# yeyupiaoling/MASR

Measured on AMD Instinct MI355X. Metric: audio-seconds/sec (RTF^-1), conformer_streaming_fbank b32x10s, PCM->fbank->encoder->ctc_greedy->text, higher is better.
Workload: dtype f32; 1 GPU; configs[1]: conformer.yml streaming fbank, batch=32 synthetic 16 kHz 10 s utterances per GPU, ctc_greedy, random-init weights V=4233; global_batch=32, parallelism=dp1, world_size_observed=1, backend=none

## Files before the change

### masr_amd/csrc/common.h

```cpp
#pragma once
#include <hip/hip_runtime.h>
#include <stdint.h>

#include "lm_scorer.h"

#ifndef MASR_EXPERIMENTS
#define MASR_EXPERIMENTS 0
#endif

typedef float f32x4 __attribute__((ext_vector_type(4)));
typedef float f32x16 __attribute__((ext_vector_type(16)));

namespace masr {

struct LdsAttr {
    size_t granted[32] = {};
};
void ensure_dynamic_lds(const void* fn, size_t bytes, LdsAttr& st);
void note_launch_error(const char* what, hipError_t e);

#ifdef __HIPCC__
struct SeqRow {
    int b, t;
};
// ... 173 lines not shown
    float eps;
};
struct FfnTail {
    const float* lnw;
    const float* lnb;
    const float* W;
    const float* bias;
    float* out;
    int N, ldo;
    const float* pre_lnw;
    const float* pre_lnb;
    long plane_stride;
    int seq_t, pad_t;
};
struct FfnHead {
    const float* glu;
    const float* dw_w;
    const float* dw_b;
    const float* lnw;
    const float* lnb;
    const float* gconst;
    const float* W;
    const float* bias;
    const int* lens;
    int seq_t, ktaps, mstride;
    float* xout;
};
int launch_ffn_fused(float* x, const float* lnw, const float* lnb, const float* w1, const float* b1, const float* w2,
                     const float* b2, int M, int dff, float eps, float scale, int affine_prologue, float* partial,
                     int nsplit, hipStream_t s, const FfnPostLn* post = nullptr, const FfnTail* tail = nullptr,
                     const FfnHead* head = nullptr, bool packed = false);
void launch_pack_ffn_pc(const float* w1, const float* w2, float* p1, float* p2, int dff, hipStream_t s);
void launch_pack_rows_pc(const float* w, float* p, int N, hipStream_t s, int n_src = -1);
int launch_ffn16(float* x, const float* lnw, const float* lnb, const float* w1, const float* b1, const float* w2, const float* b2, int M,
                 int dff, float eps, float scale, hipStream_t s, const FfnTail* tail, const FfnHead* head);
void launch_pack_ffn16(const float* w1, const float* w2, float* p1, float* p2, int dff, hipStream_t s);
void launch_pack_rows16(const float* w, float* p, int N, hipStream_t s, int n_src = -1);
struct SqzStageArgs {
    float* x;
    float* out;
    const float* att;
    const float* head_w;
    const float* head_b;
    const float *ln_a_w, *ln_a_b, *ln_b_w, *ln_b_b;
    const float *ffn_s, *ffn_b, *w1, *b1, *w2, *b2;
    const float *tail_w, *tail_b, *tail_s, *tail_sb;
    float* tail_out;
    float* glu_out;
    const float* glu;
    const float *dw_w, *dw_b, *bn_scale, *bn_shift, *gconst;
    const float* gpad;
    const int* lens;
    int M, dff, seq_t, mstride, ktaps, tail_n, glu_pad_l, glu_pad_tot;
    float eps;
    int skip_pad;
};
bool launch_sqz_stage(const SqzStageArgs& a, int stage, hipStream_t s);
#if MASR_EXPERIMENTS
int launch_ffn_dual(float* x, const float* lnw, const float* lnb, const float* p1, const float* b1, const float* p2,
                    const float* b2, int M, int dff, float eps, float scale, int affine_prologue, hipStream_t s,
                    const FfnTail* tail, const FfnHead* head);
void launch_pack_ffn_dual(const float* w1, const float* w2, float* p1, float* p2, int dff, hipStream_t s);
void launch_pack_rows_dual(const float* w, float* p, hipStream_t s);
#else
inline int launch_ffn_dual(float*, const float*, const float*, const float*, const float*, const float*, const float*, int, int, float,
                           float, int, hipStream_t, const FfnTail*, const FfnHead*) { return -1; }
inline void launch_pack_ffn_dual(const float*, const float*, float*, float*, int, hipStream_t) {}
inline void launch_pack_rows_dual(const float*, float*, hipStream_t) {}
// ... 131 lines not shown
```

### masr_amd/csrc/engine.hip

```cpp
#include <math.h>
#include <stdio.h>
#include <stdlib.h>
#include <string.h>

#include <map>
#include <mutex>
#include <string>
#include <vector>

#include "../../include/masr_hip.h"
#include "common.h"

using namespace masr;
namespace masr {
int lm_device_view(masr_lm* lm, LmView* out);
bool lm_word_based(const masr_lm* lm);
}
extern "C" const char* masr_lm_last_error(void);

static thread_local std::string g_err;
static int fail(const std::string& m) {
    g_err = m;
    return 1;
}
// ... 1030 lines not shown
        if (want_head) {
            phead = *head;
            CHK(p16(head->W, d, &phead.W));
        }
        const int done = launch_ffn16(e->x.as<float>(), lnw, lnb, it->second.first.as<float>(), b1, it->second.second.as<float>(), b2, M,
                                      dff, 1e-5f, scale, s, want_tail ? &ptail : nullptr, want_head ? &phead : nullptr);
        if (done < 0) return fail("ffn(): the 16-row FFN kernel rejected the launch");
        if (want_head && done != 4) return fail("ffn(): head stage was not launched");
        if (tail_done) *tail_done = done == 2;
        if (post_y) launch_layernorm(e->x.as<float>(), post_w, post_b, post_y, M, 1e-5f, 0, 0, nullptr, s);
        return 0;
    }
    if (packed && want_tail && tail->N % 256 == 0) {
        ptail = *tail;
        CHK(packed_rows(tail->W, tail->N, &ptail.W));
        tail = &ptail;
    }
    if (packed && want_head) {
        phead = *head;
        CHK(packed_rows(head->W, d, &phead.W));
        if (split_head) {
            CHK(e->xh.ensure((size_t)M * d * sizeof(float)));
            phead.xout = e->xh.as<float>();
        }
        head = &phead;
    }
    const int done = launch_ffn_fused(e->x.as<float>(), lnw, lnb, kw1, b1, kw2, b2, M, dff, 1e-5f, scale, affine,
                                      nsplit > 1 ? e->ffpart.as<float>() : nullptr, nsplit, s, post_y ? &post : nullptr,
                                      want_tail ? tail : nullptr, want_head ? head : nullptr, packed);
    if (done < 0) return fail("ffn(): launch rejected");
    if (want_head && !(done & 4)) return fail("ffn(): head stage was not launched");
    if (tail_done) *tail_done = done == 2;
    if (post_y && !(done & 1)) launch_layernorm(e->x.as<float>(), post_w, post_b, post_y, M, 1e-5f, 0, 0, nullptr, s);
    return 0;
}

static int g_hot_weights = 0;
static int g_embed_split = 1;
static int subsampling_conv(masr_engine* e, hipStream_t s, GemmArgs a, int amode, int nseq, const float* feats, const float* x_in) {
    const int d = e->cfg.d_model;
    const int tiles = ((a.M + 63) / 64) * ((a.N + 63) / 64);
    if (tiles >= 640 && g_conv2_rows && a.N == 256) {
        auto it = e->conv2_packed.find(a.W);
        if (it == e->conv2_packed.end()) {
            std::pair<DevBuf, DevBuf> pk;
            CHK(pk.first.ensure((size_t)a.N * a.K * sizeof(float)));
            launch_pack_conv2_rows(a.W, pk.first.as<float>(), a.K, s);
            it = e->conv2_packed.emplace(a.W, pk).first;
        }
        a.Wp = it->second.first.as<float>();
        if (feats && amode == A_CONV2 && g_conv1_fused && !g_bf16x3 && gemm_conv2_rows(a)) {
            a.feats = feats; a.mean = e->cmvn_mean; a.istd = e->cmvn_istd; a.c1w = e->conv1_w; a.c1b = e->conv1_b;
            a.Fin = e->cfg.n_mels;
        }
    }
    if (!a.feats) {
        if (feats) {
            CHK(e->x1.ensure((size_t)nseq * a.T1 * a.F1 * d * sizeof(float)));
            launch_conv1(feats, e->cmvn_mean, e->cmvn_istd, e->conv1_w, e->conv1_b, e->x1.as<float>(), nseq, a.Tin, e->cfg.n_mels,
                         d, s);
            a.A = e->x1.as<float>();
        } else {
            a.A = x_in;
        }
    }
    ProfScope ps(e, s, PROF_CONV2, 2.0 * a.M * (double)a.N * a.K);
// ... 713 lines not shown
    if (Tq_out) *Tq_out = Tq;
    return 0;
}

extern "C" {

int masr_encode_full(masr_engine* e, const float* feats_dev, const int32_t* feat_lens_dev, int32_t B, int32_t T,
                     int32_t decoding_chunk_size, float* enc_out_dev, void* stream) {
    if (!e || !e->finalized) return fail("engine not finalized");
    ENTER(e);
    CallGuard call_guard(e, (hipStream_t)stream);
    if (B <= 0) return fail("empty batch");
    hipStream_t s = (hipStream_t)stream;
    if (e->cfg.model_kind == 3) return ds2_forward(e, s, feats_dev, feat_lens_dev, B, T, enc_out_dev, nullptr, nullptr);
    const int chunk = (decoding_chunk_size > 0 && e->cfg.causal) ? decoding_chunk_size : 0;
    if (feat_lens_dev && e->input_layer != IL_CONV2D && !(feat_lens_dev = sub_lens(e, s, feat_lens_dev, B)))
        return fail("out of device memory (subsampled lengths)");
    if (e->cfg.model_kind == 1) return encode_full_squeezeformer(e, s, feats_dev, feat_lens_dev, B, T, enc_out_dev, chunk);
    if (e->cfg.model_kind == 2) return encode_full_efficient(e, s, feats_dev, feat_lens_dev, B, T, enc_out_dev, chunk);
    const int d = e->cfg.d_model, H = e->cfg.heads, pad = e->cfg.cnn_kernel - 1;
    int Tq = 0;
    CHK(embed(e, s, feats_dev, B, T, &Tq));
    if (Tq >= e->cfg.max_pos) return fail("sequence longer than max_pos");
    const int M = B * Tq;
    CHK(ensure_layer_ws(e, B, Tq));
    CHK(e->attseq.ensure(sizeof(AttSeq) * B));
    float* x = e->x.as<float>();
    EncodeCtx ctx{B, Tq, feat_lens_dev};
    launch_attseq_full(e->attseq.as<AttSeq>(), e->qkv.as<float>(), e->att.as<float>(), feat_lens_dev, B, Tq, 4, s);
    if (!e->cfg.causal)
        HIPCHK(hipMemsetAsync(e->glu.p, 0, (size_t)B * (Tq + pad) * d * sizeof(float), s));
    const LayerW* prev = nullptr;
    const bool few_rows = g_few_rows_path && (M + 31) / 32 < std::min(rowgemm_small_blocks(), g_ffn_split_blocks);
    for (const LayerW& w : e->layers) {
        const FfnTail tail{w.ln_mha_w, w.ln_mha_b, w.wqkv, w.bqkv, e->qkv.as<float>(), 3 * d, 3 * d,
                           prev ? prev->ln_fin_w : nullptr, prev ? prev->ln_fin_b : nullptr};
        bool qkv_done = false;
        CHK(ffn(e, s, M, w.ln_ffm_w, w.ln_ffm_b, w.ffm_w1, w.ffm_b1, w.ffm_w2, w.ffm_b2, 0.5f, 0, nullptr, nullptr, nullptr, &tail,
                &qkv_done));
        if (!qkv_done) mhsa(e, s, w, M);
        const bool fuse_ac = g_attn_chain && !few_rows && !g_no_chain && !e->conv_bn && H == 4 && d == 256 && g_rowgemm_packed;
        if (fuse_ac) {
            AttnChainArgs a{};
            a.seqs = e->attseq.as<AttSeq>(); a.nseq = B; a.q_stride = 3 * d; a.kv_stride = 3 * d;
            a.chunk_size = (decoding_chunk_size > 0 && e->cfg.causal) ? decoding_chunk_size : 0; a.pos_stride = 1;
            a.ptab = w.ptab; a.bias_u = w.pos_u; a.bias_v = w.pos_v;
            a.Wp = packed_rows_of(e, w.chain_w, 3 * d, s); a.bias = w.chain_b; a.lnw = w.ln_conv_w; a.lnb = w.ln_conv_b;
            a.R = x; a.R2 = x; a.C = e->glu.as<float>(); a.lens = feat_lens_dev; a.seq_t = Tq; a.mstride = 4;
            a.out_pad_l = e->cfg.causal ? pad : pad / 2; a.out_pad_tot = pad; a.eps = 1e-5f;
            if (!a.Wp) return fail("packed chain weights: allocation failed");
            ProfScope ps(e, s, PROF_ATT, 6.0 * d * (double)Tq * Tq * B + 2.0 * M * (double)(3 * d) * d);
            launch_attn_chain(a, Tq, s);
        } else {
            ProfScope ps(e, s, PROF_ATT, 6.0 * d * (double)Tq * Tq * B);
            launch_attention(e->attseq.as<AttSeq>(), B, Tq, H, 3 * d, 3 * d, w.ptab, w.pos_u, w.pos_v,
                             (decoding_chunk_size > 0 && e->cfg.causal) ? decoding_chunk_size : 0, 1, s);
        }
        if (few_rows) {
            mhsa_out(e, s, w, M);
            const bool fuse = g_split_head && e->cfg.cnn_kernel == 15 && g_ffn_packed >= 2 && !g_no_ffn_head && !e->conv_bn;
            CHK(conv_module(e, s, w, ctx, false, 0, 4, false, fuse));
            const FfnHead head{e->glu.as<float>(), w.dw_w, w.dw_b, w.cln_w, w.cln_b, e->cfg.causal ? w.gconst : nullptr,
                               w.pw2_w, w.pw2_b, feat_lens_dev, Tq, e->cfg.cnn_kernel, 4, nullptr};
            CHK(ffn(e, s, M, w.ln_ff_w, w.ln_ff_b, w.ff_w1, w.ff_b1, w.ff_w2, w.ff_b2, 0.5f, 0, w.ln_fin_w, w.ln_fin_b, x, nullptr,
                    nullptr, fuse ? &head : nullptr));
            continue;
        } else if (g_no_chain || e->conv_bn) {
            mhsa_out(e, s, w, M);
            CHK(conv_module(e, s, w, ctx, false));
            CHK(ffn(e, s, M, w.ln_ff_w, w.ln_ff_b, w.ff_w1, w.ff_b1, w.ff_w2, w.ff_b2));
        } else {
            if (!fuse_ac) mhsa_out_pw1(e, s, w, ctx);
            const FfnHead head{e->glu.as<float>(), w.dw_w, w.dw_b, w.cln_w, w.cln_b, e->cfg.causal ? w.gconst : nullptr,
                               w.pw2_w, w.pw2_b, feat_lens_dev, Tq, e->cfg.cnn_kernel, 4, nullptr};
            CHK(ffn(e, s, M, w.ln_ff_w, w.ln_ff_b, w.ff_w1, w.ff_b1, w.ff_w2, w.ff_b2, 0.5f, 0, nullptr, nullptr, nullptr, nullptr,
                    nullptr, &head));
        }
        prev = &w;
    }
    if (prev) launch_layernorm(x, prev->ln_fin_w, prev->ln_fin_b, x, M, 1e-5f, 0, 0, nullptr, s);
    launch_layernorm(x, e->after_w, e->after_b, enc_out_dev, M, 1e-5f, 0, 0, nullptr, s);
    LAUNCHCHK();
    return 0;
}

static int g_ctc_fused_blocks = 160;
static int ctc_head(masr_engine* e, const float* enc_dev, int M, float* probs_dev, int write_probs, int32_t* argmax_dev,
                    float* maxprob_dev, hipStream_t s) {
    const int d = enc_dim(e), V = e->cfg.vocab_size;
    float* logits = probs_dev;
    if (!logits) {
        CHK(e->logits.ensure((size_t)M * V * sizeof(float)));
        logits = e->logits.as<float>();
    }
    gemm(e, s, enc_dev, d, e->ctc_w, e->ctc_b, logits, V, M, V, d, ACT_NONE, 1.f, nullptr, 0);
    launch_softmax_argmax(logits, M, V, V, write_probs, argmax_dev, maxprob_dev, s);
    LAUNCHCHK();
    return 0;
}

int masr_ctc_probs(masr_engine* e, const float* enc_dev, int32_t M, float* probs_dev, int32_t* argmax_dev,
                   float* maxprob_dev, void* stream) {
    if (!e || !e->finalized) return fail("engine not finalized");
    ENTER(e);
    CallGuard call_guard(e, (hipStream_t)stream);
    if (!probs_dev) return fail("probs_dev is null");
    if (e->cfg.vocab_size > 16384) return fail("vocab_size > 16384 is not supported by the softmax / pruning kernels (one 256-thread workgroup holds a row in registers)");
    return ctc_head(e, enc_dev, M, probs_dev, 1, argmax_dev, maxprob_dev, (hipStream_t)stream);
}

int masr_ctc_greedy_frames(masr_engine* e, const float* enc_dev, int32_t M, int32_t* argmax_dev, float* maxprob_dev,
                           void* stream) {
    if (!e || !e->finalized) return fail("engine not finalized");
    ENTER(e);
// ... 1009 lines not shown
        return fail("masr_debug_set: this key selects an experimental kernel that is not in this build (MASR_BUILD_EXPERIMENTS=1)");
#endif
    if (key == 1) set_ffn_variant(value);
    else if (key == 5) g_no_chain = value;
    else if (key == 6) set_rowgemm_small(value);
    else if (key == 7) set_attention_fewq(value);
    else if (key == 14) set_attention_fold(value);
    else if (key == 15) g_embed_split = value;
    else if (key == 19) g_hot_weights = value;
    else if (key == 20) g_bf16x3 = value;
    else if (key == 21) set_gemm_bf16x3_waves(value);
    else if (key == 22) set_ffn_x3_rotation(value);
    else if (key == 23) g_ffn_packed = value;
    else if (key == 24) g_ffn_dual = value;
    else if (key == 25) g_rowgemm_packed = value;
    else if (key == 26) set_attention_grouped_fold(value);
    else if (key == 27) g_ctc_fused_blocks = value;
    else if (key == 28) set_attention_fewq_wgs(value);
    else if (key == 29) g_few_rows_path = value;
    else if (key == 30) g_split_head = value;
    else if (key == 31) g_efficient_fused = value;
    else if (key == 32) g_beam_lm_cache = value;
    else if (key == 33) set_conv2_mid_fill(value);
    else if (key == 34) g_attn_chain = value;
    else if (key == 35) g_ffn_coop = value;
    else if (key == 36) g_sqz_fused_blocks = value;
    else if (key == 37) g_beam_narrow = value;
    else if (key == 38) e->skip_padding = value;
    else if (key == 39) g_ffn16 = value;
    else if (key == 40) g_conv2_rows = value;
    else if (key == 41) g_conv1_fused = value;
    else if (key == 42) g_embed_rows = value;
    else if (key == 43) set_gru_mfma_units(value);
    else if (key == 17) set_gemm_waves(value);
    else if (key == 18) set_conv1_nt(value);
    else if (key == 16) { e->prof_stride = value > 1 ? value : 1; e->prof_seen = 0; }
    else if (key == 8) g_no_ffn_tail = value;
    else if (key == 9) g_no_ffn_head = value;
    else if (key == 12) set_rowgemm_small_blocks(value);
    else if (key == 13) g_ffn_split_blocks = value;
    else if (key == 2) {
        if (value) {
            if (!e->beam_prof) {
                void* p = nullptr;
                HIPCHK(hipMalloc(&p, 16 * sizeof(long long)));
                e->owned.push_back(p);
                e->beam_prof = (long long*)p;
            }
        } else if (e->beam_prof) {
            long long h[16];
            HIPCHK(hipMemcpy(h, e->beam_prof, sizeof(h), hipMemcpyDeviceToHost));
            fprintf(stderr, "beam phases (cycles, last workgroup): setup+hash %lld  extensions %lld  prefixes+count %lld  select %lld  compact %lld\n",
                    h[0], h[1], h[2], h[3], h[4]);
            fprintf(stderr, "  narrow step (%lld frames): tables+candidates %lld  hash+contexts %lld  children+scorer table %lld  extensions %lld  "
                    "prefixes+select %lld  scan %lld  survivors %lld  new prefixes %lld\n", h[5], h[6], h[7], h[8], h[9], h[10], h[11], h[12], h[13]);
            if (h[15] > 0) fprintf(stderr, "  wide step (%lld frames): %.1f distinct scorer contexts per frame\n", h[15], (double)h[14] / (double)h[15]);
            e->beam_prof = nullptr;
        }
    }
    else return fail("unknown debug key");
    return 0;
}

int masr_profile_select(masr_engine* e, int32_t kind) {
    if (!e) return fail("null engine");
    e->prof_kind = kind;
// ... 25 lines not shown
```

### masr_amd/csrc/ffn_pc.hip

```cpp
#include "common.h"

namespace masr {

static constexpr int PC_BM = 32;
static constexpr int PC_D = 256;
static constexpr int PC_CH = 128;
static constexpr int PC_XLD = PC_D + 4;
static constexpr int PC_HLD = PC_CH + 4;
static constexpr int PC_WLD = 32 + 4;
static constexpr int PC_WSLAB = 32 * PC_WLD;
static constexpr int PC_NSET = 4;
#ifdef PC_NOFENCE_PACKED
#define PC_FENCE(var) do { if ((var) != 2) __builtin_amdgcn_sched_barrier(0); } while (0)
#else
#define PC_FENCE(var) __builtin_amdgcn_sched_barrier(0)
#endif

#ifndef PC_BUFLOAD
#define PC_BUFLOAD 1
#endif
__device__ __forceinline__ f32x4 pc_bufld(__amdgpu_buffer_rsrc_t rs, unsigned lane16, unsigned float_index) {
    return __builtin_bit_cast(f32x4, __builtin_amdgcn_raw_buffer_load_b128(rs, lane16, float_index * 4u, 0));
}

// ... 489 lines not shown
                        } else if ((slot & 1) == 0) {
                            pre[pset][(slot - 8) >> 1] = *reinterpret_cast<const f32x4*>(
                                tsrc(t + (j + 1 + PC_NSET) / 8, (j + 1 + PC_NSET) & 7, (slot - 8) >> 1));
                        }
                        __builtin_amdgcn_sched_barrier(0);
                    }
                }
            }
            if (col < tail.N && tail.plane_stride > 0) {
                float* plane = tail.out + (size_t)t * tail.plane_stride + wave * 32 + frow;
                const int pb0 = row0 / tail.seq_t, pt0 = row0 - pb0 * tail.seq_t;
#pragma unroll
                for (int r = 0; r < 16; ++r) {
                    const int lr = (r & 3) + 8 * (r >> 2) + 4 * fh;
                    const SeqRow q = seq_row(pb0, pt0, tail.seq_t, lr);
                    if (row0 + lr < M) plane[((size_t)q.b * (tail.seq_t + tail.pad_t) + q.t) * 256] = acc[r] + bv;
                }
            } else if (col < tail.N) {
#pragma unroll
                for (int r = 0; r < 16; ++r) {
                    const int row = row0 + (r & 3) + 8 * (r >> 2) + 4 * fh;
                    if (row < M) tail.out[(size_t)row * tail.ldo + col] = acc[r] + bv;
                }
            }
        }
    }
}


static constexpr int P16_BM = 16;
static constexpr int P16_RING = 8;
__host__ __device__ constexpr int p16_k0(int kk) { return (kk & 1) * 4 + (kk >> 1); }

template <int TAIL, int HEADK>
__global__ __launch_bounds__(512) __attribute__((amdgpu_waves_per_eu(4))) void ffn16_kernel(
    float* x, const float* __restrict__ lnw, const float* __restrict__ lnb, const float* __restrict__ w1, const float* __restrict__ b1,
    const float* __restrict__ w2, const float* __restrict__ b2, int M, int dff, float eps, float scale, FfnTail tail, FfnHead head) {
    extern __shared__ __align__(16) float sm[];
    float* xn = sm;
    float* hs = xn + P16_BM * PC_XLD;

    const int tid = threadIdx.x, lane = tid & 63;
    const int wave = __builtin_amdgcn_readfirstlane(tid >> 6);
    const int role = wave >> 2, idx = wave & 3;
    const int row0 = blockIdx.x * P16_BM;
    const int fr = lane & 15, kk = lane >> 4, ko = p16_k0(kk);
    const unsigned lane16 = lane * 16;
    f32x4 pre[P16_RING];
    const float* xa = xn + fr * PC_XLD + ko;

    f32x4 gw_head = {0.f, 0.f, 0.f, 0.f}, gb_head = gw_head;
    if (HEADK > 0) {
        {
            constexpr int KT = HEADK > 0 ? HEADK : 1, pad = KT - 1;
            const int c = tid & 255, half = tid >> 8;
            float w[KT], win[KT], nw[8];
#pragma unroll
            for (int j = 0; j < KT; ++j) w[j] = head.dw_w[j * 256 + c];
            const float bv = head.dw_b[c];
            const float gc = head.gconst ? head.gconst[c] : 0.f;
            const bool has_gc = head.gconst != nullptr;
            const int hb0 = row0 / head.seq_t, ht0 = row0 - hb0 * head.seq_t, lr_last = M - 1 - row0;
#pragma unroll
            for (int rr = 0; rr < 8; ++rr) {
                const SeqRow q = seq_row(hb0, ht0, head.seq_t, min(half * 8 + rr, lr_last));
                nw[rr] = head.glu[((size_t)q.b * (pad + head.seq_t) + q.t + pad) * 256 + c];
            }
#pragma unroll
            for (int j = 0; j < KT; ++j) win[j] = 0.f;
#pragma unroll
// ... 30 lines not shown
                f32x4 o;
                o[0] = d0 * rstd * ww[0] + bb[0];
                o[1] = d1 * rstd * ww[1] + bb[1];
                o[2] = d2 * rstd * ww[2] + bb[2];
                o[3] = d3 * rstd * ww[3] + bb[3];
#pragma unroll
                for (int i = 0; i < 4; ++i) o[i] = o[i] / (1.0f + expf(-o[i]));
                *reinterpret_cast<f32x4*>(&xn[lr * PC_XLD + lane * 4]) = o;
            }
        }
        const __amdgpu_buffer_rsrc_t hrs = __builtin_amdgcn_make_buffer_rsrc(const_cast<float*>(head.W), 0, PC_D * PC_D * 4, 0x00020000);
        auto hld = [&](int f) -> f32x4 { return pc_bufld(hrs, lane16, (unsigned)(wave * 32 + f) * 256u); };
#pragma unroll
        for (int k = 0; k < P16_RING; ++k) pre[k] = hld(k);
        __syncthreads();
        {
            float bv[2], res[8];
            unsigned padded = 0;
            const int mb0 = row0 / head.seq_t, mt0 = row0 - mb0 * head.seq_t;
#pragma unroll
            for (int nt = 0; nt < 2; ++nt) {
                const int col = wave * 32 + 16 * nt + fr;
                bv[nt] = head.bias[col];
#pragma unroll
                for (int r = 0; r < 4; ++r) {
                    const int lrc = min(4 * kk + r, M - 1 - row0);
                    res[4 * nt + r] = x[(size_t)(row0 + lrc) * PC_D + col];
                    if (head.lens) {
                        const SeqRow q = seq_row(mb0, mt0, head.seq_t, lrc);
                        if (head.mstride * q.t >= head.lens[q.b]) padded |= 1u << (4 * nt + r);
                    }
                }
            }
            gw_head = *reinterpret_cast<const f32x4*>(lnw + lane * 4);
            gb_head = *reinterpret_cast<const f32x4*>(lnb + lane * 4);
            f32x4 acc[2] = {{0.f, 0.f, 0.f, 0.f}, {0.f, 0.f, 0.f, 0.f}};
            float a0 = xa[0], a1 = xa[2];
#pragma unroll
            for (int g = 0; g < 32; ++g) {
                float n0 = 0.f, n1 = 0.f;
                if (g + 1 < 32) { n0 = xa[8 * (g + 1)]; n1 = xa[8 * (g + 1) + 2]; }
#pragma unroll
                for (int q = 0; q < 4; ++q) {
                    acc[q & 1] = __builtin_amdgcn_mfma_f32_16x16x4f32(q < 2 ? a0 : a1, pre[g % P16_RING][q], acc[q & 1], 0, 0, 0);
                    if (q == 3 && g + P16_RING < 32) pre[g % P16_RING] = hld(g + P16_RING);
                    __builtin_amdgcn_sched_barrier(0);
                }
                a0 = n0;
                a1 = n1;
            }
            __syncthreads();
#pragma unroll
            for (int nt = 0; nt < 2; ++nt) {
                const int col = wave * 32 + 16 * nt + fr;
#pragma unroll
                for (int r = 0; r < 4; ++r) {
                    const int lr = 4 * kk + r;
                    float v = acc[nt][r] + bv[nt];
                    if (padded & (1u << (4 * nt + r))) v = 0.f;
                    v = res[4 * nt + r] + v;
                    if (row0 + lr < M) x[(size_t)(row0 + lr) * PC_D + col] = v;
                    xn[lr * PC_XLD + col] = v;
                }
            }
        }
        __syncthreads();
    }

    {
        const f32x4 gw = HEADK > 0 ? gw_head : *reinterpret_cast<const f32x4*>(lnw + lane * 4);
        const f32x4 gb = HEADK > 0 ? gb_head : *reinterpret_cast<const f32x4*>(lnb + lane * 4);
        f32x4 v4[2];
#pragma unroll
        for (int rr = 0; rr < 2; ++rr) {
            const int row = min(row0 + wave * 2 + rr, M - 1);
            v4[rr] = HEADK > 0 ? *reinterpret_cast<const f32x4*>(&xn[(wave * 2 + rr) * PC_XLD + lane * 4])
                               : *reinterpret_cast<const f32x4*>(x + (size_t)row * PC_D + lane * 4);
        }
        if (TAIL && tail.pre_lnw) {
            const f32x4 pw = *reinterpret_cast<const f32x4*>(tail.pre_lnw + lane * 4);
            const f32x4 pb = *reinterpret_cast<const f32x4*>(tail.pre_lnb + lane * 4);
#pragma unroll
            for (int rr = 0; rr < 2; ++rr) {
                const f32x4 v = v4[rr];
                const float mean = pc_wsum(v[0] + v[1] + v[2] + v[3]) * (1.0f / 256.0f);
                const float d0 = v[0] - mean, d1 = v[1] - mean, d2 = v[2] - mean, d3 = v[3] - mean;
                const float var = pc_wsum(d0 * d0 + d1 * d1 + d2 * d2 + d3 * d3) * (1.0f / 256.0f);
                const float rstd = 1.0f / sqrtf(var + eps);
                f32x4 o;
                o[0] = d0 * rstd * pw[0] + pb[0];
                o[1] = d1 * rstd * pw[1] + pb[1];
                o[2] = d2 * rstd * pw[2] + pb[2];
                o[3] = d3 * rstd * pw[3] + pb[3];
                v4[rr] = o;
                const int row = row0 + wave * 2 + rr;
                if (row < M) *reinterpret_cast<f32x4*>(x + (size_t)row * PC_D + lane * 4) = o;
            }
        }
#pragma unroll
        for (int rr = 0; rr < 2; ++rr) {
            const int lr = wave * 2 + rr;
            const f32x4 v = v4[rr];
            const float mean = pc_wsum(v[0] + v[1] + v[2] + v[3]) * (1.0f / 256.0f);
            const float d0 = v[0] - mean, d1 = v[1] - mean, d2 = v[2] - mean, d3 = v[3] - mean;
            const float var = pc_wsum(d0 * d0 + d1 * d1 + d2 * d2 + d3 * d3) * (1.0f / 256.0f);
            const float rstd = 1.0f / sqrtf(var + eps);
            f32x4 o;
            o[0] = d0 * rstd * gw[0] + gb[0];
            o[1] = d1 * rstd * gw[1] + gb[1];
            o[2] = d2 * rstd * gw[2] + gb[2];
            o[3] = d3 * rstd * gw[3] + gb[3];
            if (row0 + lr >= M) o = f32x4{0.f, 0.f, 0.f, 0.f};
            *reinterpret_cast<f32x4*>(&xn[lr * PC_XLD + lane * 4]) = o;
        }
    }

    const int nchunk = dff / PC_CH, nlast = nchunk - 1;
    const __amdgpu_buffer_rsrc_t wrs = __builtin_amdgcn_make_buffer_rsrc(const_cast<float*>(role == 0 ? w1 : w2), 0, dff * PC_D * 4, 0x00020000);
    auto pld = [&](int chunk, int f) -> f32x4 { return pc_bufld(wrs, lane16, (unsigned)((chunk * 4 + idx) * 32 + f) * 256u); };
#pragma unroll
    for (int k = 0; k < P16_RING; ++k) pre[k] = pld(0, k);
    __syncthreads();

    if (role == 0) {
        f32x4 accp[2] = {{0.f, 0.f, 0.f, 0.f}, {0.f, 0.f, 0.f, 0.f}};
        float bvp[2] = {0.f, 0.f};
        f32x4 resx[4];
        for (int phase = 0; phase <= nchunk + 1; ++phase) {
            float* hprev = hs + ((phase + 1) & 1) * P16_BM * PC_HLD + idx * 32 + fr;
            auto finish = [&](int e) {
                const int nt = e >> 2, r = e & 3;
                const float v = accp[nt][r] + bvp[nt];
                hprev[(4 * kk + r) * PC_HLD + 16 * nt] = v * __builtin_amdgcn_rcpf(1.0f + __expf(-v));
            };
            if (phase < nchunk) {
                const int chunk = phase;
                const float bv0 = b1[chunk * PC_CH + idx * 32 + fr], bv1 = b1[chunk * PC_CH + idx * 32 + 16 + fr];
                f32x4 acc[2] = {{0.f, 0.f, 0.f, 0.f}, {0.f, 0.f, 0.f, 0.f}};
                float a0 = xa[0], a1 = xa[2];
#pragma unroll
                for (int g = 0; g < 32; ++g) {
                    float n0 = 0.f, n1 = 0.f;
                    if (g + 1 < 32) { n0 = xa[8 * (g + 1)]; n1 = xa[8 * (g + 1) + 2]; }
#pragma unroll
                    for (int q = 0; q < 4; ++q) {
                        acc[q & 1] = __builtin_amdgcn_mfma_f32_16x16x4f32(q < 2 ? a0 : a1, pre[g % P16_RING][q], acc[q & 1], 0, 0, 0);
                        if (q == 3) pre[g % P16_RING] = pld(min(chunk + (g + P16_RING) / 32, nlast), (g + P16_RING) & 31);
                        if (phase > 0 && q == 1 && (g & 3) == 1) finish(g >> 2);
                        __builtin_amdgcn_sched_barrier(0);
                    }
                    a0 = n0;
                    a1 = n1;
                }
                accp[0] = acc[0];
                accp[1] = acc[1];
                bvp[0] = bv0;
                bvp[1] = bv1;
            } else if (phase == nchunk) {
#pragma unroll
                for (int e = 0; e < 8; ++e) finish(e);
#pragma unroll
                for (int i = 0; i < 4; ++i) {
                    const int row = min(row0 + idx * 4 + i, M - 1);
                    resx[i] = *reinterpret_cast<const f32x4*>(x + (size_t)row * PC_D + lane * 4);
                }
            } else {
#pragma unroll
                for (int i = 0; i < 4; ++i) *reinterpret_cast<f32x4*>(&xn[(idx * 4 + i) * PC_XLD + lane * 4]) = resx[i];
            }
            __syncthreads();
        }
    } else {
        f32x4 acc2[4];
#pragma unroll
        for (int n = 0; n < 4; ++n) acc2[n] = f32x4{0.f, 0.f, 0.f, 0.f};
        float bv2n[4];
#pragma unroll
        for (int n = 0; n < 4; ++n) bv2n[n] = b2[idx * 64 + 16 * n + fr];
        for (int phase = 0; phase <= nchunk + 1; ++phase) {
            if (phase >= 2) {
                const int chunk = phase - 2;
                const float* ha = hs + (phase & 1) * P16_BM * PC_HLD + fr * PC_HLD + ko;
                float a = ha[0];
#pragma unroll
                for (int f = 0; f < 32; ++f) {
                    const float an = f + 1 < 32 ? ha[8 * ((f + 1) >> 1) + 2 * ((f + 1) & 1)] : 0.f;
#pragma unroll
                    for (int q = 0; q < 4; ++q) {
                        acc2[q] = __builtin_amdgcn_mfma_f32_16x16x4f32(a, pre[f % P16_RING][q], acc2[q], 0, 0, 0);
                        if (q == 3) pre[f % P16_RING] = pld(min(chunk + (f + P16_RING) / 32, nlast), (f + P16_RING) & 31);
                        __builtin_amdgcn_sched_barrier(0);
                    }
                    a = an;
                }
            }
            __syncthreads();
        }
#pragma unroll
        for (int n = 0; n < 4; ++n) {
            const int col = idx * 64 + 16 * n + fr;
            const float bv2 = bv2n[n];
#pragma unroll
            for (int r = 0; r < 4; ++r) {
                const int lr = 4 * kk + r;
                const float v = xn[lr * PC_XLD + col] + scale * (acc2[n][r] + bv2);
                if (row0 + lr < M) x[(size_t)(row0 + lr) * PC_D + col] = v;
                if (TAIL) xn[lr * PC_XLD + col] = v;
            }
        }
    }
    if (!TAIL) return;

    {
        const f32x4 gw = *reinterpret_cast<const f32x4*>(tail.lnw + lane * 4);
        const f32x4 gb = *reinterpret_cast<const f32x4*>(tail.lnb + lane * 4);
        __syncthreads();
#pragma unroll
        for (int rr = 0; rr < 2; ++rr) {
            const int lr = wave * 2 + rr;
            const f32x4 v = *reinterpret_cast<const f32x4*>(&xn[lr * PC_XLD + lane * 4]);
            const float mean = pc_wsum(v[0] + v[1] + v[2] + v[3]) * (1.0f / 256.0f);
            const float d0 = v[0] - mean, d1 = v[1] - mean, d2 = v[2] - mean, d3 = v[3] - mean;
            const float var = pc_wsum(d0 * d0 + d1 * d1 + d2 * d2 + d3 * d3) * (1.0f / 256.0f);
            const float rstd = 1.0f / sqrtf(var + eps);
            f32x4 o;
            o[0] = d0 * rstd * gw[0] + gb[0];
            o[1] = d1 * rstd * gw[1] + gb[1];
            o[2] = d2 * rstd * gw[2] + gb[2];
            o[3] = d3 * rstd * gw[3] + gb[3];
            if (row0 + lr >= M) o = f32x4{0.f, 0.f, 0.f, 0.f};
            *reinterpret_cast<f32x4*>(&xn[lr * PC_XLD + lane * 4]) = o;
        }
    }
    const int ntile = (tail.N + 255) / 256;
    const __amdgpu_buffer_rsrc_t trs = __builtin_amdgcn_make_buffer_rsrc(const_cast<float*>(tail.W), 0, ntile * 256 * PC_D * 4, 0x00020000);
    auto tld = [&](int t, int f) -> f32x4 { return pc_bufld(trs, lane16, (unsigned)((min(t, ntile - 1) * 8 + wave) * 32 + f) * 256u); };
#pragma unroll
    for (int k = 0; k < P16_RING; ++k) pre[k] = tld(0, k);
    __syncthreads();
    for (int t = 0; t < ntile; ++t) {
// ... 38 lines not shown
        }
    }
}

__global__ __launch_bounds__(256) void pack_ffn16_kernel(const float* __restrict__ w1, const float* __restrict__ w2,
                                                         float* __restrict__ p1, float* __restrict__ p2, int dff) {
    const size_t n = (size_t)dff * PC_D;
    const size_t t = (size_t)blockIdx.x * 256 + threadIdx.x;
    if (t >= 2 * n) return;
    const bool second = t >= n;
    const size_t e = second ? t - n : t;
    const int q = (int)(e & 3), lane = (int)((e >> 2) & 63), f = (int)((e >> 8) & 31), idx = (int)((e >> 13) & 3), chunk = (int)(e >> 15);
    const int fr = lane & 15, ko = p16_k0(lane >> 4);
    if (!second) p1[e] = w1[(size_t)(chunk * PC_CH + 32 * idx + 16 * (q & 1) + fr) * PC_D + 8 * f + ko + 2 * (q >> 1)];
    else p2[e] = w2[(size_t)(64 * idx + 16 * q + fr) * dff + chunk * PC_CH + 8 * (f >> 1) + ko + 2 * (f & 1)];
}
__global__ __launch_bounds__(256) void pack_rows16_kernel(const float* __restrict__ w, float* __restrict__ p, int N, int n_src) {
    const size_t e = (size_t)blockIdx.x * 256 + threadIdx.x;
    if (e >= (size_t)N * PC_D) return;
    const int q = (int)(e & 3), lane = (int)((e >> 2) & 63), f = (int)((e >> 8) & 31), wave = (int)((e >> 13) & 7), t = (int)(e >> 16);
    const int row = t * 256 + 32 * wave + 16 * (q & 1) + (lane & 15);
    p[e] = row < n_src ? w[(size_t)row * PC_D + 8 * f + p16_k0(lane >> 4) + 2 * (q >> 1)] : 0.f;
}
void launch_pack_ffn16(const float* w1, const float* w2, float* p1, float* p2, int dff, hipStream_t s) {
    const size_t n = (size_t)2 * dff * PC_D;
    hipLaunchKernelGGL(pack_ffn16_kernel, dim3((unsigned)((n + 255) / 256)), dim3(256), 0, s, w1, w2, p1, p2, dff);
}
void launch_pack_rows16(const float* w, float* p, int N, hipStream_t s, int n_src) {
    const size_t n = (size_t)N * PC_D;
    hipLaunchKernelGGL(pack_rows16_kernel, dim3((unsigned)((n + 255) / 256)), dim3(256), 0, s, w, p, N, n_src < 0 ? N : n_src);
}

int launch_ffn16(float* x, const float* lnw, const float* lnb, const float* w1, const float* b1, const float* w2, const float* b2, int M,
                 int dff, float eps, float scale, hipStream_t s, const FfnTail* tail, const FfnHead* head) {
    if (M <= 0) return 0;
    if (dff % PC_CH || dff <= 0 || (tail && tail->out && head && head->glu)) return -1;
    const size_t lds = (size_t)(P16_BM * PC_XLD + 2 * P16_BM * PC_HLD) * sizeof(float);
    const dim3 grid((M + P16_BM - 1) / P16_BM);
    if (head && head->glu) {
        if (head->ktaps == 15)
            hipLaunchKernelGGL((ffn16_kernel<0, 15>), grid, dim3(512), lds, s, x, lnw, lnb, w1, b1, w2, b2, M, dff, eps, scale, FfnTail{}, *head);
        else if (head->ktaps == 7)
            hipLaunchKernelGGL((ffn16_kernel<0, 7>), grid, dim3(512), lds, s, x, lnw, lnb, w1, b1, w2, b2, M, dff, eps, scale, FfnTail{}, *head);
        else
            return -1;
        return 4;
    }
    if (tail && tail->out) {
        if (tail->N % 256) return -1;
        hipLaunchKernelGGL((ffn16_kernel<1, 0>), grid, dim3(512), lds, s, x, lnw, lnb, w1, b1, w2, b2, M, dff, eps, scale, *tail, FfnHead{});
        return 2;
    }
    hipLaunchKernelGGL((ffn16_kernel<0, 0>), grid, dim3(512), lds, s, x, lnw, lnb, w1, b1, w2, b2, M, dff, eps, scale, FfnTail{}, FfnHead{});
    return 0;
}

__global__ __launch_bounds__(64) void mfma_order_probe_kernel(const float* __restrict__ a, const float* __restrict__ b, float* c32,
                                                              float* c16, int K, int4 p0, int4 p1) {
    const int lane = threadIdx.x;
    {
        const int frow = lane & 31, fh = lane >> 5;
        f32x16 acc;
#pragma unroll
        for (int r = 0; r < 16; ++r) acc[r] = 0.f;
        for (int g = 0; g < K / 8; ++g)
#pragma unroll
            for (int q = 0; q < 4; ++q) {
                const int k = 8 * g + 4 * fh + q;
                const float av = frow < 16 ? a[frow * K + k] : 0.f, bv = frow < 16 ? b[frow * K + k] : 0.f;
                acc = __builtin_amdgcn_mfma_f32_32x32x2f32(av, bv, acc, 0, 0, 0);
            }
#pragma unroll
        for (int r = 0; r < 16; ++r) {
            const int row = (r & 3) + 8 * (r >> 2) + 4 * fh;
            if (row < 16 && frow < 16) c32[row * 16 + frow] = acc[r];
        }
    }
    {
        const int fr = lane & 15, kk = lane >> 4;
        const int o0 = kk == 0 ? p0.x : kk == 1 ? p0.y : kk == 2 ? p0.z : p0.w;
        const int o1 = kk == 0 ? p1.x : kk == 1 ? p1.y : kk == 2 ? p1.z : p1.w;
        f32x4 acc = {0.f, 0.f, 0.f, 0.f};
        for (int g = 0; g < K / 8; ++g) {
            acc = __builtin_amdgcn_mfma_f32_16x16x4f32(a[fr * K + 8 * g + o0], b[fr * K + 8 * g + o0], acc, 0, 0, 0);
            acc = __builtin_amdgcn_mfma_f32_16x16x4f32(a[fr * K + 8 * g + o1], b[fr * K + 8 * g + o1], acc, 0, 0, 0);
        }
// ... 113 lines not shown
```

Measured before the change: 52560 audio-seconds/sec.

## Fuse layer-end FFN with next layer's macaron FFN and QKV tail in one kernel

Adds a joint path where a single ffn16 kernel launch runs the conv-module head, the current layer's second FFN, the next layer's first (macaron) FFN and the QKV projection tail. Rows stay in LDS between the two FFN passes, so the intermediate write and re-read of x and one kernel launch per layer boundary go away. For the last layer, the final and after layernorms are fused into the kernel epilogue, replacing two separate layernorm launches. In exchange the kernel grows more complex (a pass loop and kernarg pointer tricks), which risks register pressure and lower occupancy, and each block runs longer.

```diff
diff --git a/masr_amd/csrc/common.h b/masr_amd/csrc/common.h
--- a/masr_amd/csrc/common.h
+++ b/masr_amd/csrc/common.h
@@ -229,8 +229,14 @@
                      const FfnHead* head = nullptr, bool packed = false);
 void launch_pack_ffn_pc(const float* w1, const float* w2, float* p1, float* p2, int dff, hipStream_t s);
 void launch_pack_rows_pc(const float* w, float* p, int N, hipStream_t s, int n_src = -1);
+struct FfnNext {
+    const float *lnw, *lnb, *w1, *b1, *w2, *b2;
+    float scale;
+    const float *fin_w, *fin_b, *after_w, *after_b;
+    float* enc_out;
+};
 int launch_ffn16(float* x, const float* lnw, const float* lnb, const float* w1, const float* b1, const float* w2, const float* b2, int M,
-                 int dff, float eps, float scale, hipStream_t s, const FfnTail* tail, const FfnHead* head);
+                 int dff, float eps, float scale, hipStream_t s, const FfnTail* tail, const FfnHead* head, const FfnNext* next = nullptr);
 void launch_pack_ffn16(const float* w1, const float* w2, float* p1, float* p2, int dff, hipStream_t s);
 void launch_pack_rows16(const float* w, float* p, int N, hipStream_t s, int n_src = -1);
 struct SqzStageArgs {
diff --git a/masr_amd/csrc/engine.hip b/masr_amd/csrc/engine.hip
--- a/masr_amd/csrc/engine.hip
+++ b/masr_amd/csrc/engine.hip
@@ -1086,6 +1086,55 @@
     if (want_head && !(done & 4)) return fail("ffn(): head stage was not launched");
     if (tail_done) *tail_done = done == 2;
     if (post_y && !(done & 1)) launch_layernorm(e->x.as<float>(), post_w, post_b, post_y, M, 1e-5f, 0, 0, nullptr, s);
+    return 0;
+}
+
+static int g_layer_joint = 1;
+static int ffn16_layer_joint(masr_engine* e, hipStream_t s, int M, const LayerW& w, const LayerW* nw, const FfnHead& head, float* enc_out) {
+    const int d = e->cfg.d_model, dff = e->cfg.d_ff;
+    auto rows16 = [&](const float* W, int N, const float** out) -> int {
+        auto it = e->ffn16_packed.find(W);
+        if (it == e->ffn16_packed.end()) {
+            std::pair<DevBuf, DevBuf> pk;
+            CHK(pk.first.ensure((size_t)N * d * sizeof(float)));
+            launch_pack_rows16(W, pk.first.as<float>(), N, s);
+            it = e->ffn16_packed.emplace(W, pk).first;
+        }
+        *out = it->second.first.as<float>();
+        return 0;
+    };
+    auto ffn16 = [&](const float* w1, const float* w2, const float** p1, const float** p2) -> int {
+        auto it = e->ffn16_packed.find(w1);
+        if (it == e->ffn16_packed.end()) {
+            std::pair<DevBuf, DevBuf> pk;
+            CHK(pk.first.ensure((size_t)dff * d * sizeof(float)));
+            CHK(pk.second.ensure((size_t)dff * d * sizeof(float)));
+            launch_pack_ffn16(w1, w2, pk.first.as<float>(), pk.second.as<float>(), dff, s);
+            it = e->ffn16_packed.emplace(w1, pk).first;
+        }
+        *p1 = it->second.first.as<float>();
+        *p2 = it->second.second.as<float>();
+        return 0;
+    };
+    const float *p1, *p2;
+    CHK(ffn16(w.ff_w1, w.ff_w2, &p1, &p2));
+    FfnHead phead = head;
+    CHK(rows16(head.W, d, &phead.W));
+    FfnNext next{};
+    FfnTail tail{};
+    if (nw) {
+        CHK(ffn16(nw->ffm_w1, nw->ffm_w2, &next.w1, &next.w2));
+        next.lnw = nw->ln_ffm_w; next.lnb = nw->ln_ffm_b; next.b1 = nw->ffm_b1; next.b2 = nw->ffm_b2; next.scale = 0.5f;
+        tail = FfnTail{nw->ln_mha_w, nw->ln_mha_b, nullptr, nw->bqkv, e->qkv.as<float>(), 3 * d, 3 * d, w.ln_fin_w, w.ln_fin_b};
+        CHK(rows16(nw->wqkv, 3 * d, &tail.W));
+    } else {
+        next.fin_w = w.ln_fin_w; next.fin_b = w.ln_fin_b; next.after_w = e->after_w; next.after_b = e->after_b; next.enc_out = enc_out;
+    }
+    const double f_ffn = 4.0 * M * (double)dff * d;
+    ProfScope ps(e, s, nw ? PROF_FFN_TAIL : PROF_FFN_HEAD, f_ffn + 2.0 * M * (double)d * d + (nw ? f_ffn + 2.0 * M * (double)(3 * d) * d : 0.0));
+    const int done = launch_ffn16(e->x.as<float>(), w.ln_ff_w, w.ln_ff_b, p1, w.ff_b1, p2, w.ff_b2, M, dff, 1e-5f, 0.5f, s, nw ? &tail : nullptr,
+                                  &phead, &next);
+    if (done != (nw ? 6 : 4)) return fail("ffn16_layer_joint(): the 16-row FFN kernel rejected the launch");
     return 0;
 }
 
@@ -1865,13 +1914,22 @@
         HIPCHK(hipMemsetAsync(e->glu.p, 0, (size_t)B * (Tq + pad) * d * sizeof(float), s));
     const LayerW* prev = nullptr;
     const bool few_rows = g_few_rows_path && (M + 31) / 32 < std::min(rowgemm_small_blocks(), g_ffn_split_blocks);
-    for (const LayerW& w : e->layers) {
-        const FfnTail tail{w.ln_mha_w, w.ln_mha_b, w.wqkv, w.bqkv, e->qkv.as<float>(), 3 * d, 3 * d,
-                           prev ? prev->ln_fin_w : nullptr, prev ? prev->ln_fin_b : nullptr};
-        bool qkv_done = false;
-        CHK(ffn(e, s, M, w.ln_ffm_w, w.ln_ffm_b, w.ffm_w1, w.ffm_b1, w.ffm_w2, w.ffm_b2, 0.5f, 0, nullptr, nullptr, nullptr, &tail,
-                &qkv_done));
-        if (!qkv_done) mhsa(e, s, w, M);
+    const bool joint = g_layer_joint && !few_rows && !g_no_chain && !e->conv_bn && (M + 31) / 32 >= g_ffn_split_blocks && d == 256 &&
+                       g_ffn_packed && g_ffn16 && !g_ffn_dual && !(g_bf16x3 & 2) && !g_no_ffn_tail && !g_no_ffn_head &&
+                       e->cfg.d_ff % 128 == 0 && (e->cfg.cnn_kernel == 15 || e->cfg.cnn_kernel == 7);
+    bool ffn1_done = false;
+    bool closed = false;
+    for (size_t li = 0; li < e->layers.size(); ++li) {
+        const LayerW& w = e->layers[li];
+        if (!ffn1_done) {
+            const FfnTail tail{w.ln_mha_w, w.ln_mha_b, w.wqkv, w.bqkv, e->qkv.as<float>(), 3 * d, 3 * d,
+                               prev ? prev->ln_fin_w : nullptr, prev ? prev->ln_fin_b : nullptr};
+            bool qkv_done = false;
+            CHK(ffn(e, s, M, w.ln_ffm_w, w.ln_ffm_b, w.ffm_w1, w.ffm_b1, w.ffm_w2, w.ffm_b2, 0.5f, 0, nullptr, nullptr, nullptr, &tail,
+                    &qkv_done));
+            if (!qkv_done) mhsa(e, s, w, M);
+        }
+        ffn1_done = false;
         const bool fuse_ac = g_attn_chain && !few_rows && !g_no_chain && !e->conv_bn && H == 4 && d == 256 && g_rowgemm_packed;
         if (fuse_ac) {
             AttnChainArgs a{};
@@ -1906,13 +1964,22 @@
             if (!fuse_ac) mhsa_out_pw1(e, s, w, ctx);
             const FfnHead head{e->glu.as<float>(), w.dw_w, w.dw_b, w.cln_w, w.cln_b, e->cfg.causal ? w.gconst : nullptr,
                                w.pw2_w, w.pw2_b, feat_lens_dev, Tq, e->cfg.cnn_kernel, 4, nullptr};
-            CHK(ffn(e, s, M, w.ln_ff_w, w.ln_ff_b, w.ff_w1, w.ff_b1, w.ff_w2, w.ff_b2, 0.5f, 0, nullptr, nullptr, nullptr, nullptr,
-                    nullptr, &head));
+            if (joint) {
+                const LayerW* nw = li + 1 < e->layers.size() ? &e->layers[li + 1] : nullptr;
+                CHK(ffn16_layer_joint(e, s, M, w, nw, head, enc_out_dev));
+                ffn1_done = nw != nullptr;
+                closed = nw == nullptr;
+            } else {
+                CHK(ffn(e, s, M, w.ln_ff_w, w.ln_ff_b, w.ff_w1, w.ff_b1, w.ff_w2, w.ff_b2, 0.5f, 0, nullptr, nullptr, nullptr, nullptr,
+                        nullptr, &head));
+            }
         }
         prev = &w;
     }
-    if (prev) launch_layernorm(x, prev->ln_fin_w, prev->ln_fin_b, x, M, 1e-5f, 0, 0, nullptr, s);
-    launch_layernorm(x, e->after_w, e->after_b, enc_out_dev, M, 1e-5f, 0, 0, nullptr, s);
+    if (!closed) {
+        if (prev) launch_layernorm(x, prev->ln_fin_w, prev->ln_fin_b, x, M, 1e-5f, 0, 0, nullptr, s);
+        launch_layernorm(x, e->after_w, e->after_b, enc_out_dev, M, 1e-5f, 0, 0, nullptr, s);
+    }
     LAUNCHCHK();
     return 0;
 }
@@ -2988,6 +3055,7 @@
     else if (key == 41) g_conv1_fused = value;
     else if (key == 42) g_embed_rows = value;
     else if (key == 43) set_gru_mfma_units(value);
+    else if (key == 44) g_layer_joint = value;
     else if (key == 17) set_gemm_waves(value);
     else if (key == 18) set_conv1_nt(value);
     else if (key == 16) { e->prof_stride = value > 1 ? value : 1; e->prof_seen = 0; }
diff --git a/masr_amd/csrc/ffn_pc.hip b/masr_amd/csrc/ffn_pc.hip
--- a/masr_amd/csrc/ffn_pc.hip
+++ b/masr_amd/csrc/ffn_pc.hip
@@ -545,10 +545,34 @@
 static constexpr int P16_RING = 8;
 __host__ __device__ constexpr int p16_k0(int kk) { return (kk & 1) * 4 + (kk >> 1); }
 
-template <int TAIL, int HEADK>
+struct Ffn16Pass {
+    const float *lnw, *lnb, *w1, *b1, *w2, *b2;
+    float scale;
+};
+struct Ffn16Next {
+    Ffn16Pass pass[2];
+    const float *fin_w, *fin_b, *after_w, *after_b;
+    float* enc_out;
+};
+
+struct Ffn16KArgs {
+    float* x;
+    const float *lnw, *lnb, *w1, *b1, *w2, *b2;
+    int M, dff;
+    float eps, scale;
+    FfnTail tail;
+    FfnHead head;
+    Ffn16Next next;
+};
+
+template <int TAIL, int HEADK, int JOINT>
 __global__ __launch_bounds__(512) __attribute__((amdgpu_waves_per_eu(4))) void ffn16_kernel(
     float* x, const float* __restrict__ lnw, const float* __restrict__ lnb, const float* __restrict__ w1, const float* __restrict__ b1,
-    const float* __restrict__ w2, const float* __restrict__ b2, int M, int dff, float eps, float scale, FfnTail tail, FfnHead head) {
+    const float* __restrict__ w2, const float* __restrict__ b2, int M, int dff, float eps, float scale, FfnTail tail_arg, FfnHead head, Ffn16Next next_arg) {
+    static_assert(!JOINT || (TAIL && HEADK > 0), "the joint launch runs head, two FFNs and tail");
+    const char* kargs = (const char*)__builtin_amdgcn_kernarg_segment_ptr();
+    const FfnTail& tail = JOINT ? *(const FfnTail*)(kargs + offsetof(Ffn16KArgs, tail)) : tail_arg;
+    const Ffn16Next& next = *(const Ffn16Next*)(kargs + offsetof(Ffn16KArgs, next));
     extern __shared__ __align__(16) float sm[];
     float* xn = sm;
     float* hs = xn + P16_BM * PC_XLD;
@@ -645,8 +669,10 @@
                     }
                 }
             }
-            gw_head = *reinterpret_cast<const f32x4*>(lnw + lane * 4);
-            gb_head = *reinterpret_cast<const f32x4*>(lnb + lane * 4);
+            if (!JOINT) {
+                gw_head = *reinterpret_cast<const f32x4*>(lnw + lane * 4);
+                gb_head = *reinterpret_cast<const f32x4*>(lnb + lane * 4);
+            }
             f32x4 acc[2] = {{0.f, 0.f, 0.f, 0.f}, {0.f, 0.f, 0.f, 0.f}};
             float a0 = xa[0], a1 = xa[2];
 #pragma unroll
@@ -680,9 +706,30 @@
         __syncthreads();
     }
 
+    const bool closing = HEADK > 0 && !TAIL && next.enc_out != nullptr;
+    const int nchunk = dff / PC_CH, nlast = nchunk - 1;
+#pragma clang loop unroll(disable)
+    for (int pass = 0; pass < (JOINT ? 2 : 1); ++pass) {
+    const bool second = JOINT && pass == 1;
+    float* xq = x;
+    int rq = row0;
+    if (JOINT) asm volatile("" : "+s"(xq), "+s"(rq));
+    float* const x = xq;
+    const int row0 = rq;
+    const float* c_lnw = JOINT ? next.pass[pass].lnw : lnw;
+    const float* c_lnb = JOINT ? next.pass[pass].lnb : lnb;
+    const float* c_w1 = JOINT ? next.pass[pass].w1 : w1;
+    const float* c_b1 = JOINT ? next.pass[pass].b1 : b1;
+    const float* c_w2 = JOINT ? next.pass[pass].w2 : w2;
+    const float* c_b2 = JOINT ? next.pass[pass].b2 : b2;
+    const float c_scale = JOINT ? next.pass[pass].scale : scale;
+    if (second) __syncthreads();
     {
-        const f32x4 gw = HEADK > 0 ? gw_head : *reinterpret_cast<const f32x4*>(lnw + lane * 4);
-        const f32x4 gb = HEADK > 0 ? gb_head : *reinterpret_cast<const f32x4*>(lnb + lane * 4);
+        f32x4 gw = gw_head, gb = gb_head;
+        if (HEADK == 0 || JOINT) {
+            gw = *reinterpret_cast<const f32x4*>(c_lnw + lane * 4);
+            gb = *reinterpret_cast<const f32x4*>(c_lnb + lane * 4);
+        }
         f32x4 v4[2];
 #pragma unroll
         for (int rr = 0; rr < 2; ++rr) {
@@ -690,7 +737,7 @@
             v4[rr] = HEADK > 0 ? *reinterpret_cast<const f32x4*>(&xn[(wave * 2 + rr) * PC_XLD + lane * 4])
                                : *reinterpret_cast<const f32x4*>(x + (size_t)row * PC_D + lane * 4);
         }
-        if (TAIL && tail.pre_lnw) {
+        if (TAIL && tail.pre_lnw && (!JOINT || second)) {
             const f32x4 pw = *reinterpret_cast<const f32x4*>(tail.pre_lnw + lane * 4);
             const f32x4 pb = *reinterpret_cast<const f32x4*>(tail.pre_lnb + lane * 4);
 #pragma unroll
@@ -728,8 +775,7 @@
         }
     }
 
-    const int nchunk = dff / PC_CH, nlast = nchunk - 1;
-    const __amdgpu_buffer_rsrc_t wrs = __builtin_amdgcn_make_buffer_rsrc(const_cast<float*>(role == 0 ? w1 : w2), 0, dff * PC_D * 4, 0x00020000);
+    const __amdgpu_buffer_rsrc_t wrs = __builtin_amdgcn_make_buffer_rsrc(const_cast<float*>(role == 0 ? c_w1 : c_w2), 0, dff * PC_D * 4, 0x00020000);
     auto pld = [&](int chunk, int f) -> f32x4 { return pc_bufld(wrs, lane16, (unsigned)((chunk * 4 + idx) * 32 + f) * 256u); };
 #pragma unroll
     for (int k = 0; k < P16_RING; ++k) pre[k] = pld(0, k);
@@ -748,7 +794,7 @@
             };
             if (phase < nchunk) {
                 const int chunk = phase;
-                const float bv0 = b1[chunk * PC_CH + idx * 32 + fr], bv1 = b1[chunk * PC_CH + idx * 32 + 16 + fr];
+                const float bv0 = c_b1[chunk * PC_CH + idx * 32 + fr], bv1 = c_b1[chunk * PC_CH + idx * 32 + 16 + fr];
                 f32x4 acc[2] = {{0.f, 0.f, 0.f, 0.f}, {0.f, 0.f, 0.f, 0.f}};
                 float a0 = xa[0], a1 = xa[2];
 #pragma unroll
@@ -789,7 +835,7 @@
         for (int n = 0; n < 4; ++n) acc2[n] = f32x4{0.f, 0.f, 0.f, 0.f};
         float bv2n[4];
 #pragma unroll
-        for (int n = 0; n < 4; ++n) bv2n[n] = b2[idx * 64 + 16 * n + fr];
+        for (int n = 0; n < 4; ++n) bv2n[n] = c_b2[idx * 64 + 16 * n + fr];
         for (int phase = 0; phase <= nchunk + 1; ++phase) {
             if (phase >= 2) {
                 const int chunk = phase - 2;
@@ -816,9 +862,37 @@
 #pragma unroll
             for (int r = 0; r < 4; ++r) {
                 const int lr = 4 * kk + r;
-                const float v = xn[lr * PC_XLD + col] + scale * (acc2[n][r] + bv2);
-                if (row0 + lr < M) x[(size_t)(row0 + lr) * PC_D + col] = v;
-                if (TAIL) xn[lr * PC_XLD + col] = v;
+                const float v = xn[lr * PC_XLD + col] + c_scale * (acc2[n][r] + bv2);
+                if (row0 + lr < M && !(JOINT && !second) && !closing) x[(size_t)(row0 + lr) * PC_D + col] = v;
+                if (TAIL || closing) xn[lr * PC_XLD + col] = v;
+            }
+        }
+    }
+    }
+    if (closing) {
+        const f32x4 fw = *reinterpret_cast<const f32x4*>(next.fin_w + lane * 4);
+        const f32x4 fb = *reinterpret_cast<const f32x4*>(next.fin_b + lane * 4);
+        const f32x4 aw = *reinterpret_cast<const f32x4*>(next.after_w + lane * 4);
+        const f32x4 ab = *reinterpret_cast<const f32x4*>(next.after_b + lane * 4);
+        __syncthreads();
+#pragma unroll
+        for (int rr = 0; rr < 2; ++rr) {
+            const int lr = wave * 2 + rr, row = row0 + lr;
+            f32x4 v = *reinterpret_cast<const f32x4*>(&xn[lr * PC_XLD + lane * 4]);
+#pragma unroll
+            for (int st = 0; st < 2; ++st) {
+                const f32x4 w4 = st ? aw : fw, b4 = st ? ab : fb;
+                const float mean = pc_wsum(v[0] + v[1] + v[2] + v[3]) * (1.0f / 256.0f);
+                const float d0 = v[0] - mean, d1 = v[1] - mean, d2 = v[2] - mean, d3 = v[3] - mean;
+                const float var = pc_wsum(d0 * d0 + d1 * d1 + d2 * d2 + d3 * d3) * (1.0f / 256.0f);
+                const float rstd = 1.0f / sqrtf(var + eps);
+                f32x4 o;
+                o[0] = d0 * rstd * w4[0] + b4[0];
+                o[1] = d1 * rstd * w4[1] + b4[1];
+                o[2] = d2 * rstd * w4[2] + b4[2];
+                o[3] = d3 * rstd * w4[3] + b4[3];
+                v = o;
+                if (row < M) *reinterpret_cast<f32x4*>((st ? next.enc_out : x) + (size_t)row * PC_D + lane * 4) = o;
             }
         }
     }
@@ -923,26 +997,45 @@
 }
 
 int launch_ffn16(float* x, const float* lnw, const float* lnb, const float* w1, const float* b1, const float* w2, const float* b2, int M,
-                 int dff, float eps, float scale, hipStream_t s, const FfnTail* tail, const FfnHead* head) {
+                 int dff, float eps, float scale, hipStream_t s, const FfnTail* tail, const FfnHead* head, const FfnNext* next) {
     if (M <= 0) return 0;
-    if (dff % PC_CH || dff <= 0 || (tail && tail->out && head && head->glu)) return -1;
+    const bool has_tail = tail && tail->out, has_head = head && head->glu, joint = next && next->w1;
+    if (dff % PC_CH || dff <= 0 || (has_tail && has_head) != joint || (joint && (!tail->pre_lnw || next->enc_out))) return -1;
+    if (next && next->enc_out && !has_head) return -1;
     const size_t lds = (size_t)(P16_BM * PC_XLD + 2 * P16_BM * PC_HLD) * sizeof(float);
     const dim3 grid((M + P16_BM - 1) / P16_BM);
-    if (head && head->glu) {
+    Ffn16Next nx{};
+    if (joint) {
+        nx.pass[0] = Ffn16Pass{lnw, lnb, w1, b1, w2, b2, scale};
+        nx.pass[1] = Ffn16Pass{next->lnw, next->lnb, next->w1, next->b1, next->w2, next->b2, next->scale};
+    } else if (next) {
+        nx.fin_w = next->fin_w; nx.fin_b = next->fin_b; nx.after_w = next->after_w; nx.after_b = next->after_b; nx.enc_out = next->enc_out;
+    }
+    if (joint) {
+        if (tail->N % 256) return -1;
         if (head->ktaps == 15)
-            hipLaunchKernelGGL((ffn16_kernel<0, 15>), grid, dim3(512), lds, s, x, lnw, lnb, w1, b1, w2, b2, M, dff, eps, scale, FfnTail{}, *head);
+            hipLaunchKernelGGL((ffn16_kernel<1, 15, 1>), grid, dim3(512), lds, s, x, lnw, lnb, w1, b1, w2, b2, M, dff, eps, scale, *tail, *head, nx);
         else if (head->ktaps == 7)
-            hipLaunchKernelGGL((ffn16_kernel<0, 7>), grid, dim3(512), lds, s, x, lnw, lnb, w1, b1, w2, b2, M, dff, eps, scale, FfnTail{}, *head);
+            hipLaunchKernelGGL((ffn16_kernel<1, 7, 1>), grid, dim3(512), lds, s, x, lnw, lnb, w1, b1, w2, b2, M, dff, eps, scale, *tail, *head, nx);
+        else
+            return -1;
+        return 6;
+    }
+    if (has_head) {
+        if (head->ktaps == 15)
+            hipLaunchKernelGGL((ffn16_kernel<0, 15, 0>), grid, dim3(512), lds, s, x, lnw, lnb, w1, b1, w2, b2, M, dff, eps, scale, FfnTail{}, *head, nx);
+        else if (head->ktaps == 7)
+            hipLaunchKernelGGL((ffn16_kernel<0, 7, 0>), grid, dim3(512), lds, s, x, lnw, lnb, w1, b1, w2, b2, M, dff, eps, scale, FfnTail{}, *head, nx);
         else
             return -1;
         return 4;
     }
-    if (tail && tail->out) {
+    if (has_tail) {
         if (tail->N % 256) return -1;
-        hipLaunchKernelGGL((ffn16_kernel<1, 0>), grid, dim3(512), lds, s, x, lnw, lnb, w1, b1, w2, b2, M, dff, eps, scale, *tail, FfnHead{});
+        hipLaunchKernelGGL((ffn16_kernel<1, 0, 0>), grid, dim3(512), lds, s, x, lnw, lnb, w1, b1, w2, b2, M, dff, eps, scale, *tail, FfnHead{}, nx);
         return 2;
     }
-    hipLaunchKernelGGL((ffn16_kernel<0, 0>), grid, dim3(512), lds, s, x, lnw, lnb, w1, b1, w2, b2, M, dff, eps, scale, FfnTail{}, FfnHead{});
+    hipLaunchKernelGGL((ffn16_kernel<0, 0, 0>), grid, dim3(512), lds, s, x, lnw, lnb, w1, b1, w2, b2, M, dff, eps, scale, FfnTail{}, FfnHead{}, nx);
     return 0;
 }
 
```

Result: no change. 52780 audio-seconds/sec (median of 6 runs) (+0.4%).
